# thangvubk/SoftGroup

Measured on AMD Instinct MI355X. Metric: scans/sec ScanNet-v2-like inference (softgroup_scannet.yaml, full forward_test), higher is better.
Workload: dtype f32

## Files before the change

### softgroup_amd/csrc/ballquery.hip

```cpp
#include "common.h"
#include "scan.h"

namespace sg {

constexpr int32_t kBqEmpty = 0x7f7f7f7f;
constexpr int kBqBuf = 2048;
constexpr int kBqCap = SG_BALLQUERY_MAX_NEIGHBORS;
constexpr int kBqKeep = 64;

struct BqWs {
  int4 *cell;
  int32_t *table;
  int32_t *count;
  int32_t *start;
  int32_t *cursor;
  int32_t *slot_of;
  float4 *sorted;
  int32_t *keep;
  void *scan_ws;
  size_t scan_bytes;
  uint32_t cap;
};

__device__ __forceinline__ uint32_t cell_slot(int b, int cx, int cy, int cz, uint32_t mask) {
  uint64_t h = (static_cast<uint64_t>(static_cast<uint32_t>(b)) << 32) | static_cast<uint32_t>(cx);
  h = mix64(h) ^ ((static_cast<uint64_t>(static_cast<uint32_t>(cy)) << 32) | static_cast<uint32_t>(cz));
  return static_cast<uint32_t>(mix64(h)) & mask;
}

__global__ void __launch_bounds__(256) bq_insert_kernel(const float *__restrict__ xyz,
                                                       const int32_t *__restrict__ batch_idxs,
                                                       int n, double inv_cell, int4 *__restrict__ cell,
                                                       int32_t *table, uint32_t mask, int32_t *count,
                                                       int32_t *__restrict__ slot_of) {
  const int i = blockIdx.x * 256 + threadIdx.x;
  if (i >= n) return;
  int4 c;
  c.x = batch_idxs ? batch_idxs[i] : 0;
  c.y = static_cast<int>(floor(static_cast<double>(xyz[3 * i + 0]) * inv_cell));
  c.z = static_cast<int>(floor(static_cast<double>(xyz[3 * i + 1]) * inv_cell));
  c.w = static_cast<int>(floor(static_cast<double>(xyz[3 * i + 2]) * inv_cell));
  cell[i] = c;
  uint32_t s = cell_slot(c.x, c.y, c.z, c.w, mask);
  while (true) {
    int32_t cur = __hip_atomic_load(&table[s], __ATOMIC_RELAXED, __HIP_MEMORY_SCOPE_AGENT);
    if (cur == kBqEmpty) {
      cur = atomicCAS(&table[s], kBqEmpty, i);
      if (cur == kBqEmpty) break;
    }
    int4 o;
    o.x = batch_idxs ? batch_idxs[cur] : 0;
    o.y = static_cast<int>(floor(static_cast<double>(xyz[3 * cur + 0]) * inv_cell));
    o.z = static_cast<int>(floor(static_cast<double>(xyz[3 * cur + 1]) * inv_cell));
    o.w = static_cast<int>(floor(static_cast<double>(xyz[3 * cur + 2]) * inv_cell));
    if (o.x == c.x && o.y == c.y && o.z == c.z && o.w == c.w) break;
    s = (s + 1) & mask;
  }
  slot_of[i] = static_cast<int32_t>(s);
  atomicAdd(&count[s], 1);
}

__global__ void __launch_bounds__(256) bq_scatter_kernel(const float *__restrict__ xyz, int n,
                                                        const int32_t *__restrict__ slot_of,
                                                        const int32_t *__restrict__ start,
                                                        int32_t *cursor, float4 *__restrict__ sorted) {
  const int i = blockIdx.x * 256 + threadIdx.x;
  if (i >= n) return;
  const int s = slot_of[i];
  const int pos = start[s] + atomicAdd(&cursor[s], 1);
  sorted[pos] = make_float4(xyz[3 * i], xyz[3 * i + 1], xyz[3 * i + 2], __int_as_float(i));
}

__device__ __forceinline__ float dist2(float ox, float oy, float oz, float x, float y, float z) {
  const float dx = __fsub_rn(ox, x), dy = __fsub_rn(oy, y), dz = __fsub_rn(oz, z);
  return __fmaf_rn(dz, dz, __fmaf_rn(dx, dx, __fmul_rn(dy, dy)));
}

struct BqCells {
  int start, excl, incl, total;
};
__device__ __forceinline__ BqCells bq_cells(int my_start, int my_count) {
  BqCells c;
  c.start = my_start;
  c.incl = wave_incl_scan(my_count);
  c.excl = c.incl - my_count;
  c.total = __shfl(c.incl, 63, 64);
  return c;
}
__device__ __forceinline__ int bq_candidate(const BqCells &c, int t) {
  int lo = 0, hi = 26;
#pragma unroll
  for (int it = 0; it < 5; ++it) {
    const int mid = (lo + hi) >> 1;
    const bool right = __shfl(c.incl, mid, 64) <= t;
    lo = right ? mid + 1 : lo;
    hi = right ? hi : mid;
  }
  return __shfl(c.start, lo, 64) + (t - __shfl(c.excl, lo, 64));
}

__device__ __forceinline__ int bq_scan_count(const float4 *__restrict__ sorted, const BqCells &c,
                                             float ox, float oy, float oz, float r2, int limit) {
  int total = 0;
  for (int t0 = 0; t0 < c.total; t0 += 64) {
    const int t = t0 + lane_id();
    const int at = bq_candidate(c, min(t, c.total - 1));
    if (t < c.total) {
      const float4 p = sorted[at];
      total += (dist2(ox, oy, oz, p.x, p.y, p.z) < r2 && __float_as_int(p.w) < limit) ? 1 : 0;
    }
  }
  return wave_sum(total);
}

template <bool FILL>
__global__ void __launch_bounds__(256) bq_query_kernel(const float *__restrict__ xyz, int n,
                                                      float r2, const int4 *__restrict__ cell,
                                                      const int32_t *__restrict__ table,
                                                      const int32_t *__restrict__ count,
                                                      const int32_t *__restrict__ start,
                                                      uint32_t mask, const float4 *__restrict__ sorted,
                                                      int32_t *__restrict__ start_len,
                                                      int32_t *__restrict__ idx_out, int32_t *__restrict__ keep) {
  __shared__ __attribute__((aligned(16))) int32_t buf_all[FILL ? 4 * kBqBuf : 4 * kBqKeep];
  const int wave = threadIdx.x >> 6, lane = threadIdx.x & 63;
  int32_t *buf = buf_all + wave * (FILL ? kBqBuf : kBqKeep);
  for (int i = blockIdx.x * 4 + wave; i < n; i += gridDim.x * 4) {
    if (FILL) {
      const int out_len = start_len[2 * i + 1];
      if (out_len <= kBqKeep) {
        if (lane < out_len) idx_out[static_cast<int64_t>(start_len[2 * i]) + lane] = keep[static_cast<int64_t>(i) * kBqKeep + lane];
        continue;
      }
    }
    const float ox = xyz[3 * i], oy = xyz[3 * i + 1], oz = xyz[3 * i + 2];
    const int4 c = cell[i];
    int my_start = 0, my_count = 0;
    if (lane < 27) {
      const int cx = c.y + lane / 9 - 1, cy = c.z + (lane / 3) % 3 - 1, cz = c.w + lane % 3 - 1;
      uint32_t s = cell_slot(c.x, cx, cy, cz, mask);
      while (true) {
        const int32_t rep = table[s];
        if (rep == kBqEmpty) break;
        const int4 o = cell[rep];
        if (o.x == c.x && o.y == cx && o.z == cy && o.w == cz) {
          my_start = start[s];
          my_count = count[s];
          break;
        }
        s = (s + 1) & mask;
      }
    }
    const BqCells cells = bq_cells(my_start, my_count);
    if (!FILL) {
      int m = 0;
      for (int t0 = 0; t0 < cells.total; t0 += 64) {
        const int t = t0 + lane;
        const int at = bq_candidate(cells, min(t, cells.total - 1));
        bool ok = false;
        int id = 0;
        if (t < cells.total) {
          const float4 p = sorted[at];
          id = __float_as_int(p.w);
          ok = dist2(ox, oy, oz, p.x, p.y, p.z) < r2;
        }
        const uint64_t bal = __ballot(ok);
        const int pos = m + mask_prefix(bal);
        if (ok && pos < kBqKeep) buf[pos] = id;
        m += __popcll(bal);
      }
      if (lane == 0) start_len[2 * i + 1] = min(m, kBqCap);
      if (m <= kBqKeep) {
        __builtin_amdgcn_fence(__ATOMIC_RELEASE, "wavefront");
        __builtin_amdgcn_wave_barrier();
        const int e = lane < m ? buf[lane] : 0x7fffffff;
        int rank = 0;
        for (int j = 0; j < m; ++j) rank += (buf[j] < e);
        if (lane < m) keep[static_cast<int64_t>(i) * kBqKeep + rank] = e;
      }
      __builtin_amdgcn_wave_barrier();
      continue;
    }
    const int out_start = start_len[2 * i], out_len = start_len[2 * i + 1];
    int limit = 0x7fffffff;
    int m = 0;
    for (int attempt = 0; attempt < 2; ++attempt) {
      m = 0;
      for (int t0 = 0; t0 < cells.total; t0 += 64) {
        const int t = t0 + lane;
        const int at = bq_candidate(cells, min(t, cells.total - 1));
        bool ok = false;
        int id = 0;
        if (t < cells.total) {
          const float4 p = sorted[at];
          id = __float_as_int(p.w);
          ok = dist2(ox, oy, oz, p.x, p.y, p.z) < r2 && id < limit;
        }
        const uint64_t bal = __ballot(ok);
        const int pos = m + mask_prefix(bal);
        if (ok && pos < kBqBuf) buf[pos] = id;
        m += __popcll(bal);
      }
      if (m <= kBqBuf) break;
      int lo = 0, hi = n;
      while (lo < hi) {
        const int mid = lo + (hi - lo) / 2;
        const int cmid = bq_scan_count(sorted, cells, ox, oy, oz, r2, mid);
        if (cmid >= out_len) hi = mid; else lo = mid + 1;
      }
      limit = lo;
    }
    __builtin_amdgcn_fence(__ATOMIC_RELEASE, "wavefront");
    __builtin_amdgcn_wave_barrier();
    for (int e0 = 0; e0 < m; e0 += 64) {
      const int ei = e0 + lane;
      const int e = ei < m ? buf[ei] : 0x7fffffff;
      int rank = 0;
      int j = 0;
      for (; j + 4 <= m; j += 4) {
        const int4 q = *reinterpret_cast<const int4 *>(buf + j);
        rank += (q.x < e) + (q.y < e) + (q.z < e) + (q.w < e);
      }
      for (; j < m; ++j) rank += (buf[j] < e);
      if (ei < m && rank < out_len) idx_out[static_cast<int64_t>(out_start) + rank] = e;
    }
    __builtin_amdgcn_wave_barrier();
  }
}

static size_t bq_cap(int n) {
  size_t cap = 1024;
  while (cap < static_cast<size_t>(n) * 2) cap <<= 1;
  return cap;
}

static bool bq_carve(void *ws, size_t ws_bytes, int n, BqWs *w) {
  Workspace a(ws, ws_bytes);
  const size_t nn = static_cast<size_t>(n > 0 ? n : 1);
  w->cap = static_cast<uint32_t>(bq_cap(n));
  w->cell = a.take<int4>(nn);
  w->sorted = a.take<float4>(nn);
  w->table = a.take<int32_t>(w->cap);
  w->count = a.take<int32_t>(w->cap);
  w->start = a.take<int32_t>(w->cap);
  w->cursor = a.take<int32_t>(w->cap);
  w->slot_of = a.take<int32_t>(nn);
  w->scan_bytes = scan_workspace_bytes(w->cap);
  w->scan_ws = a.take<char>(w->scan_bytes);
  w->keep = a.take<int32_t>(nn * kBqKeep);
  return w->scan_ws != nullptr && w->keep != nullptr;
}

}

using namespace sg;

extern "C" {

size_t sg_ballquery_workspace_bytes(int n) {
  const size_t nn = static_cast<size_t>(n > 0 ? n : 1);
  const size_t cap = bq_cap(n);
  return 2 * align_up(nn * 16) + 4 * align_up(cap * 4) + align_up(nn * 4) +
         align_up(scan_workspace_bytes(cap)) + align_up(nn * kBqKeep * 4) + 256;
}

int sg_ballquery_build_grid(const float *xyz, const int32_t *batch_idxs, int n, float radius,
                            void *ws, size_t ws_bytes, sg_stream_t stream_) {
  SG_REQUIRE(n >= 0 && radius > 0.f, "sg_ballquery_build_grid: bad arguments (n=%d r=%g)", n, radius);
  hipStream_t stream = as_stream(stream_);
  BqWs w;
  if (!bq_carve(ws, ws_bytes, n, &w)) {
    set_error("sg_ballquery_build_grid: workspace too small");
    return SG_ERR_WORKSPACE;
  }
  if (n == 0) return SG_OK;
  {
    FillList f;
    f.add(w.table, static_cast<size_t>(w.cap) * 4, 0x7f);
    f.add(w.count, static_cast<size_t>(w.cap) * 4, 0);
    f.add(w.cursor, static_cast<size_t>(w.cap) * 4, 0);
    fill_many(f, stream);
  }
  const double inv_cell = 1.0 / (static_cast<double>(radius) * (1.0 + 1e-6));
  const int grid = (n + 255) / 256;
  bq_insert_kernel<<<grid, 256, 0, stream>>>(xyz, batch_idxs, n, inv_cell, w.cell, w.table,
                                             w.cap - 1, w.count, w.slot_of);
  const int32_t *count = w.count;
  int32_t *start = w.start;
  auto in = [count] __device__(int64_t s) { return count[s]; };
  auto out = [start] __device__(int64_t s, int v) { start[s] = v; };
  int rc = exclusive_scan(in, out, w.cap, nullptr, w.scan_ws, w.scan_bytes, stream);
  if (rc != SG_OK) return rc;
  bq_scatter_kernel<<<grid, 256, 0, stream>>>(xyz, n, w.slot_of, w.start, w.cursor, w.sorted);
  return check_launch("sg_ballquery_build_grid");
}

int sg_ballquery_count(const float *xyz, const int32_t *batch_idxs, int n, float radius,
                       int32_t *start_len, int32_t *meta, void *ws, size_t ws_bytes,
                       sg_stream_t stream_) {
  (void)batch_idxs;
  (void)meta;
  SG_REQUIRE(n >= 0 && radius > 0.f, "sg_ballquery_count: bad arguments");
  BqWs w;
  if (!bq_carve(ws, ws_bytes, n, &w)) {
    set_error("sg_ballquery_count: workspace too small");
    return SG_ERR_WORKSPACE;
  }
  if (n == 0) return SG_OK;
  const float r2 = radius * radius;
  bq_query_kernel<false><<<grid_for(n, 4, 256 * 16), 256, 0, as_stream(stream_)>>>(
      xyz, n, r2, w.cell, w.table, w.count, w.start, w.cap - 1, w.sorted, start_len, nullptr, w.keep);
  return check_launch("sg_ballquery_count");
}

int sg_ballquery_fill(const float *xyz, const int32_t *batch_idxs, int n, float radius,
                      const int32_t *start_len, int32_t *idx, void *ws, size_t ws_bytes,
                      sg_stream_t stream_) {
  (void)batch_idxs;
  SG_REQUIRE(n >= 0 && radius > 0.f, "sg_ballquery_fill: bad arguments");
  BqWs w;
  if (!bq_carve(ws, ws_bytes, n, &w)) {
    set_error("sg_ballquery_fill: workspace too small");
    return SG_ERR_WORKSPACE;
  }
  if (n == 0) return SG_OK;
  const float r2 = radius * radius;
  bq_query_kernel<true><<<grid_for(n, 4, 256 * 16), 256, 0, as_stream(stream_)>>>(
      xyz, n, r2, w.cell, w.table, w.count, w.start, w.cap - 1, w.sorted,
      const_cast<int32_t *>(start_len), idx, w.keep);
  return check_launch("sg_ballquery_fill");
}

}
```

### softgroup_amd/csrc/bfs.hip

```cpp
#include <stdlib.h>

#include <map>
#include <mutex>
#include <utility>

#include "common.h"
#include "scan.h"

namespace sg {

constexpr int kCap = SG_BALLQUERY_MAX_NEIGHBORS;
constexpr int kEmitThreads = 512;
constexpr int kEmitWaves = kEmitThreads / 64;

#define SG_LD(p) __hip_atomic_load((p), __ATOMIC_RELAXED, __HIP_MEMORY_SCOPE_AGENT)
#define SG_ST(p, v) __hip_atomic_store((p), (v), __ATOMIC_RELAXED, __HIP_MEMORY_SCOPE_AGENT)

struct BfsWs {
  int32_t *parent, *lab, *size, *cid, *coff, *owner, *seeds, *ebase, *wcnt, *asym_nodes;
  int4 *label;
  int2 *erec;
  int32_t *counters;
  void *scan_ws;
  size_t scan_bytes;
// ... 1 lines not shown
  unsigned long long *big_rec[2];
};

constexpr int kBigFastWgs = 16;
constexpr int kBigSlice = 8192;
constexpr int kBigClusterMin = 16384;
inline bool big_fast_on() {
  const char *e = getenv("SG_BFS_BIG_FAST");
  return !(e && atoi(e) == 0);
}
inline int thin_levels_on() {
  const char *e = getenv("SG_BFS_THIN");
  return e ? atoi(e) : 0;
}
inline bool big_local_on() {
  const char *e = getenv("SG_BFS_BIG_LOCAL");
  return !(e && atoi(e) == 0);
}
inline size_t big_stage_entries(int n) {
  return n > kBigClusterMin && big_fast_on() ? static_cast<size_t>(n) + static_cast<size_t>(kBigFastWgs) * kBigSlice : 0;
}

static bool bfs_carve(void *ws, size_t ws_bytes, int n, int64_t n_edges, BfsWs *w) {
  Workspace a(ws, ws_bytes);
  const size_t nn = static_cast<size_t>(n > 0 ? n : 1);
  w->parent = a.take<int32_t>(nn);
  w->lab = a.take<int32_t>(nn);
  w->label = a.take<int4>(nn);
  w->size = a.take<int32_t>(nn);
  w->cid = a.take<int32_t>(nn);
  w->coff = a.take<int32_t>(nn);
  w->owner = a.take<int32_t>(nn);
  w->seeds = a.take<int32_t>(nn);
  w->ebase = a.take<int32_t>(nn);
  w->wcnt = a.take<int32_t>(nn);
  w->asym_nodes = a.take<int32_t>(nn);
  w->counters = a.take<int32_t>(64);
  w->scan_bytes = scan_workspace_bytes(n);
  w->scan_ws = a.take<char>(w->scan_bytes);
  w->erec = a.take<int2>(static_cast<size_t>(n_edges > 0 ? n_edges : 1));
  bool ok = w->scan_ws != nullptr && w->erec != nullptr;
  const size_t be = big_stage_entries(n);
  for (int i = 0; i < 2; ++i) {
    w->big_stage[i] = be ? a.take<int32_t>(be) : nullptr;
    w->big_rec[i] = be ? a.take<unsigned long long>(be) : nullptr;
    ok = ok && (be == 0 || (w->big_stage[i] != nullptr && w->big_rec[i] != nullptr));
  }
  return ok;
}

__device__ __forceinline__ int uf_find(int32_t *parent, int x) {
  int cur = SG_LD(&parent[x]);
  if (cur != x) {
    int prev = x, next;
    while (cur > (next = SG_LD(&parent[cur]))) {
      SG_ST(&parent[prev], next);
      prev = cur;
      cur = next;
    }
  }
  return cur;
}

__device__ __forceinline__ void uf_union(int32_t *parent, int a, int b) {
  while (a != b) {
    if (a < b) { const int t = a; a = b; b = t; }
    const int old = atomicCAS(&parent[a], a, b);
    if (old == a) return;
    a = uf_find(parent, old);
    b = uf_find(parent, b);
  }
}

__device__ __forceinline__ bool list_has_sorted(const int32_t *__restrict__ lst, int len, int key) {
  int lo = 0, hi = len;
  while (lo < hi) {
    const int mid = (lo + hi) >> 1;
    const int v = lst[mid];
    if (v < key) lo = mid + 1; else hi = mid;
  }
  return lo < len && lst[lo] == key;
}

__global__ void __launch_bounds__(256) bfs_init_kernel(int n, int32_t *parent, int32_t *size,
                                                      int32_t *owner) {
  const int i = blockIdx.x * 256 + threadIdx.x;
  if (i < n) {
    parent[i] = i;
    size[i] = 0;
    owner[i] = 0x7fffffff;
  }
}

constexpr int kSample = 2;
template <int SAMPLE>
__global__ void __launch_bounds__(256) bfs_union_kernel(const int32_t *__restrict__ idx,
                                                       const int32_t *__restrict__ start_len, int n,
                                                       int lists_sorted, int radius_lists,
                                                       int32_t *parent, int32_t *asym_nodes,
                                                       int32_t *counters) {
  const int wave = threadIdx.x >> 6, lane = threadIdx.x & 63;
  for (int u = blockIdx.x * 4 + wave; u < n; u += gridDim.x * 4) {
    const int st = start_len[2 * u], ln_all = start_len[2 * u + 1];
    const int ln = SAMPLE ? min(ln_all, kSample) : ln_all;
    const bool u_capped = ln_all >= kCap;
    bool any_asym = false;
    const int ru = SAMPLE ? -1 : SG_LD(&parent[u]);
    for (int p0 = 0; p0 < ln; p0 += 64) {
      const int p = p0 + lane;
      const int v = p < ln ? idx[st + p] : u;
      bool sym = true;
      if (v != u) {
        const int vst = start_len[2 * v], vln = start_len[2 * v + 1];
        if (!radius_lists || u_capped || vln >= kCap) {
          if (lists_sorted) {
            sym = list_has_sorted(idx + vst, vln, u);
          } else {
            sym = false;
            for (int j = 0; j < vln; ++j)
              if (idx[vst + j] == u) { sym = true; break; }
          }
        }
        if (sym) {
          if (v < u && (SAMPLE || SG_LD(&parent[v]) != ru)) uf_union(parent, uf_find(parent, u), uf_find(parent, v));
        }
      }
      any_asym |= !sym;
    }
    if (!SAMPLE && __any(any_asym)) {
      if (lane == 0) asym_nodes[atomicAdd(&counters[0], 1)] = u;
    }
  }
}

__global__ void __launch_bounds__(256) bfs_hook_min_kernel(const int32_t *__restrict__ idx,
                                                          const int32_t *__restrict__ start_len, int n,
                                                          int lists_sorted, int radius_lists, int32_t *parent) {
  const int u = blockIdx.x * 256 + threadIdx.x;
  if (u >= n) return;
  const int st = start_len[2 * u], ln = start_len[2 * u + 1];
  if (ln == 0 || !lists_sorted) return;
  const int v = idx[st];
  if (v >= u) return;
  if (!radius_lists || ln >= kCap || start_len[2 * v + 1] >= kCap)
    if (!list_has_sorted(idx + start_len[2 * v], start_len[2 * v + 1], u)) return;
  parent[u] = v;
}
__global__ void __launch_bounds__(256) bfs_compress_kernel(int n, int32_t *parent) {
  const int i = blockIdx.x * 256 + threadIdx.x;
  if (i < n) SG_ST(&parent[i], uf_find(parent, i));
}

__global__ void __launch_bounds__(256) bfs_flatten_kernel(int n, int32_t *parent, int32_t *lab) {
  const int i = blockIdx.x * 256 + threadIdx.x;
  if (i >= n) return;
  int r = i;
  while (true) {
    const int p = SG_LD(&parent[r]);
    if (p == r) break;
    r = p;
  }
  lab[i] = r;
}
__global__ void __launch_bounds__(256) bfs_store_root_kernel(int n, const int32_t *__restrict__ lab,
                                                            int32_t *__restrict__ parent) {
  const int i = blockIdx.x * 256 + threadIdx.x;
  if (i < n) parent[i] = lab[i];
}

__global__ void __launch_bounds__(256) bfs_propagate_kernel(const int32_t *__restrict__ idx,
                                                           const int32_t *__restrict__ start_len,
                                                           const int32_t *__restrict__ asym_nodes,
                                                           int n_asym,
                                                           const int32_t *__restrict__ root_of,
                                                           int32_t *lab, int32_t *counters) {
  const int wave = threadIdx.x >> 6, lane = threadIdx.x & 63;
  for (int a = blockIdx.x * 4 + wave; a < n_asym; a += gridDim.x * 4) {
    const int u = asym_nodes[a];
    const int ru = root_of[u];
    const int st = start_len[2 * u], ln = start_len[2 * u + 1];
    for (int p = lane; p < ln; p += 64) {
      const int rv = root_of[idx[st + p]];
      if (rv == ru) continue;
      const int lu = SG_LD(&lab[ru]);
      if (lu < SG_LD(&lab[rv])) {
        if (atomicMin(&lab[rv], lu) > lu) SG_ST(&counters[1], 1);
      }
    }
  }
}

__global__ void __launch_bounds__(256) bfs_label_kernel(int n, const int32_t *__restrict__ root_of,
                                                       const int32_t *__restrict__ lab,
                                                       const int32_t *__restrict__ start_len,
                                                       int4 *__restrict__ node_rec, int32_t *size) {
  const int i = blockIdx.x * 256 + threadIdx.x;
  const bool valid = i < n;
  const int l = valid ? lab[root_of[i]] : -1;
  int slot = 0;
  uint64_t todo = __ballot(valid);
  const int lane = threadIdx.x & 63;
  while (todo) {
    const int leader = __ffsll(static_cast<long long>(todo)) - 1;
    const int ll = __shfl(l, leader, 64);
    const uint64_t same = __ballot(valid && l == ll) & todo;
    int base = 0;
    if (lane == leader) base = atomicAdd(&size[ll], __popcll(same));
    base = __shfl(base, leader, 64);
    if ((same >> lane) & 1ull) slot = base + __popcll(same & ((1ull << lane) - 1ull));
    todo &= ~same;
  }
  if (!valid) return;
  node_rec[i] = make_int4(l, slot, start_len[2 * i], start_len[2 * i + 1]);
}

__global__ void __launch_bounds__(256) bfs_zero_size_kernel(int n, int32_t *size) {
  const int i = blockIdx.x * 256 + threadIdx.x;
  if (i < n) size[i] = 0;
}

__global__ void __launch_bounds__(256) bfs_owner_reset_kernel(int n, const int4 *__restrict__ label,
                                                             const int32_t *__restrict__ size,
                                                             int min_size, const int32_t *gate,
                                                             int32_t *__restrict__ owner) {
  if (SG_LD(gate) == 0) return;
  for (int i = blockIdx.x * 256 + threadIdx.x; i < n; i += gridDim.x * 256)
    if (size[label[i].x] > min_size) owner[i] = 0x7fffffff;
// ... 1321 lines not shown
    hipStreamDestroy(it->second.side);
    hipEventDestroy(it->second.fork);
    hipEventDestroy(it->second.join);
    hipEventDestroy(it->second.back);
  }
  g_bfs_side.erase(it);
}
struct BfsLabelNote {
  const void *ws = nullptr;
  int max_kept = -1;
};
static thread_local BfsLabelNote t_bfs_note;

void bfs_emit_defer(BfsDefer *d) { t_bfs_defer = d; }
int bfs_emit_join(const BfsDefer &d, hipStream_t stream) {
  if (!d.deferred) return SG_OK;
  BfsSide *side = bfs_side(stream);
  if (side == nullptr || side->side != d.side || hipEventRecord(side->join, side->side) != hipSuccess ||
      hipStreamWaitEvent(stream, side->join, 0) != hipSuccess) {
    set_error("bfs_emit_join: joining the side stream failed");
    return SG_ERR_LAUNCH;
  }
  return SG_OK;
}
int bfs_label_max_kept(const void *ws) { return t_bfs_note.ws == ws ? t_bfs_note.max_kept : -1; }

__global__ void __launch_bounds__(256) bfs_kept_members_kernel(const int32_t *__restrict__ l2p, int n_pts,
                                                              const int4 *__restrict__ label,
                                                              const int32_t *__restrict__ size,
                                                              const float *__restrict__ thr_dev,
                                                              int32_t *__restrict__ out) {
  __shared__ int wsum[4];
  const float thr = thr_dev[0];
  int mine = 0;
  for (int p = blockIdx.x * 256 + threadIdx.x; p < n_pts; p += gridDim.x * 256)
    mine += static_cast<float>(size[label[l2p[p]].x]) >= thr ? 1 : 0;
  const int w = wave_sum(mine);
  if ((threadIdx.x & 63) == 0) wsum[threadIdx.x >> 6] = w;
  __syncthreads();
  if (threadIdx.x == 0) atomicAdd(out, wsum[0] + wsum[1] + wsum[2] + wsum[3]);
}
int bfs_count_kept_members(const void *ws, size_t ws_bytes, int n, int64_t n_edges, const int32_t *l2p, int n_pts,
                           const float *thr_dev, int32_t *out, hipStream_t stream) {
  BfsWs w;
  if (!bfs_carve(const_cast<void *>(ws), ws_bytes, n, n_edges, &w)) {
    set_error("bfs_count_kept_members: workspace too small");
    return SG_ERR_WORKSPACE;
  }
  hipMemsetAsync(out, 0, 4, stream);
  bfs_kept_members_kernel<<<grid_for(n_pts, 256, 1024), 256, 0, stream>>>(l2p, n_pts, w.label, w.size, thr_dev, out);
  return check_launch("bfs_count_kept_members");
}

}

using namespace sg;

extern "C" {

size_t sg_bfs_workspace_bytes(int n, int64_t n_edges) {
  const size_t nn = static_cast<size_t>(n > 0 ? n : 1);
  const size_t ne = static_cast<size_t>(n_edges > 0 ? n_edges : 1);
  const size_t be = big_stage_entries(n);
  return 14 * align_up(nn * 4) + align_up(64 * 4) + align_up(scan_workspace_bytes(n)) +
         align_up(ne * sizeof(int2)) + 2 * (align_up(be * 4) + align_up(be * 8)) + 256;
}

int sg_bfs_cluster_label(const int32_t *bq_idxs, const int32_t *start_len, int n, int64_t n_edges,
                         int list_flags, const int32_t *seg_of_point, const float *seg_thr,
                         int n_seg, int32_t *n_cluster_host, int32_t *sum_npoint_host, void *ws,
                         size_t ws_bytes, sg_stream_t stream_) {
  SG_REQUIRE(n >= 0 && n_seg >= 1 && seg_thr != nullptr, "sg_bfs_cluster_label: bad arguments");
  hipStream_t stream = as_stream(stream_);
  BfsWs w;
  if (!bfs_carve(ws, ws_bytes, n, n_edges, &w)) {
    set_error("sg_bfs_cluster_label: workspace too small");
    return SG_ERR_WORKSPACE;
  }
  *n_cluster_host = 0;
  *sum_npoint_host = 0;
  if (n == 0) return SG_OK;
  const int grid = (n + 255) / 256;
  hipMemsetAsync(w.counters, 0, 64 * 4, stream);
  bfs_init_kernel<<<grid, 256, 0, stream>>>(n, w.parent, w.size, w.owner);
  static const bool one_pass = getenv("SG_BFS_ONE_PASS") != nullptr;
  if (!one_pass) {
    static const bool sample_env = getenv("SG_BFS_SAMPLE") != nullptr;
    if (sample_env || !(list_flags & SG_LISTS_SORTED))
      bfs_union_kernel<1><<<grid_for(n, 4, 256 * 16), 256, 0, stream>>>(bq_idxs, start_len, n,
                                                                      list_flags & SG_LISTS_SORTED,
                                                                      list_flags & SG_LISTS_RADIUS,
                                                                      w.parent, w.asym_nodes, w.counters);
    else
      bfs_hook_min_kernel<<<grid, 256, 0, stream>>>(bq_idxs, start_len, n, list_flags & SG_LISTS_SORTED,
                                                   list_flags & SG_LISTS_RADIUS, w.parent);
    bfs_compress_kernel<<<grid, 256, 0, stream>>>(n, w.parent);
  }
  bfs_union_kernel<0><<<grid_for(n, 4, 256 * 16), 256, 0, stream>>>(bq_idxs, start_len, n,
                                                                  list_flags & SG_LISTS_SORTED,
                                                                  list_flags & SG_LISTS_RADIUS,
                                                                  w.parent, w.asym_nodes, w.counters);
  bfs_flatten_kernel<<<grid, 256, 0, stream>>>(n, w.parent, w.lab);
  bfs_store_root_kernel<<<grid, 256, 0, stream>>>(n, w.lab, w.parent);

  int32_t *host_counters = pinned_words();
  SG_REQUIRE(host_counters != nullptr, "sg_bfs_cluster_label: pinned allocation failed");
  for (int i = 0; i < 5; ++i) host_counters[i] = 0;
  for (int pass = 0; pass < 2; ++pass) {
    if (pass == 1) {
      const int n_asym = host_counters[0];
      while (true) {
        hipMemsetAsync(w.counters + 1, 0, 4, stream);
        bfs_propagate_kernel<<<grid_for(n_asym, 4, 256 * 16), 256, 0, stream>>>(
            bq_idxs, start_len, w.asym_nodes, n_asym, w.parent, w.lab, w.counters);
        host_counters[8] = 0;
        hipMemcpyAsync(host_counters + 8, w.counters + 1, 4, hipMemcpyDeviceToHost, stream);
        if (hipStreamSynchronize(stream) != hipSuccess) return check_launch("bfs propagate");
        if (!host_counters[8]) break;
      }
      bfs_zero_size_kernel<<<grid, 256, 0, stream>>>(n, w.size);
    }
    bfs_label_kernel<<<grid, 256, 0, stream>>>(n, w.parent, w.lab, start_len, w.label, w.size);
    const int4 *label = w.label;
    const int32_t *size = w.size;
    int32_t *cid = w.cid, *coff = w.coff;
    auto keep = [label, size, seg_of_point, seg_thr] __device__(int64_t i) -> int {
      if (label[i].x != static_cast<int32_t>(i)) return 0;
      const float thr = seg_thr[seg_of_point ? seg_of_point[i] : 0];
      return static_cast<float>(size[i]) >= thr ? 1 : 0;
    };
    int32_t *max_kept = w.counters + 4;
    auto keep_size = [keep, size, max_kept] __device__(int64_t i) -> int {
      const int s = keep(i) ? size[i] : 0;
      if (s > kBigMin) atomicMax(max_kept, s);
      return s;
    };
    int rc = exclusive_scan(keep, [cid] __device__(int64_t i, int v) { cid[i] = v; }, n,
                            w.counters + 2, w.scan_ws, w.scan_bytes, stream);
    if (rc != SG_OK) return rc;
    rc = exclusive_scan(keep_size, [coff] __device__(int64_t i, int v) { coff[i] = v; }, n,
                        w.counters + 3, w.scan_ws, w.scan_bytes, stream);
    if (rc != SG_OK) return rc;
    hipMemcpyAsync(host_counters, w.counters, 5 * sizeof(int32_t), hipMemcpyDeviceToHost, stream);
    if (hipStreamSynchronize(stream) != hipSuccess) return check_launch("sg_bfs_cluster_label");
    if (host_counters[0] == 0) break;
    if (pass == 0) hipMemsetAsync(w.counters + 4, 0, 4, stream);
  }
  *n_cluster_host = host_counters[2];
  *sum_npoint_host = host_counters[3];
  t_bfs_note.ws = ws;
  t_bfs_note.max_kept = host_counters[4];
  return check_launch("sg_bfs_cluster_label");
}

int sg_bfs_cluster_emit(const int32_t *bq_idxs, const int32_t *start_len, int n, int64_t n_edges,
                        const int32_t *seg_of_point, const float *seg_thr, int n_cluster,
                        int sum_npoint, int32_t *cluster_idxs, int32_t *cluster_offsets, void *ws,
                        size_t ws_bytes, sg_stream_t stream_) {
  SG_REQUIRE(n >= 0 && n_cluster >= 0 && sum_npoint >= 0, "sg_bfs_cluster_emit: bad arguments");
  hipStream_t stream = as_stream(stream_);
  BfsWs w;
  if (!bfs_carve(ws, ws_bytes, n, n_edges, &w)) {
    set_error("sg_bfs_cluster_emit: workspace too small");
    return SG_ERR_WORKSPACE;
  }
  if (n_cluster == 0 || n == 0) {
    hipMemsetAsync(cluster_offsets, 0, 4, stream);
    return SG_OK;
  }
  bfs_seed_kernel<<<(n + 255) / 256, 256, 0, stream>>>(n, w.label, w.size, w.cid, w.coff,
                                                       seg_of_point, seg_thr, w.seeds,
                                                       cluster_offsets);
  bfs_edge_rec_kernel<<<grid_for(n, 4, 256 * 16), 256, 0, stream>>>(bq_idxs, w.label, w.cid, w.seeds, n,
                                                                     n_cluster, w.erec);
  static const bool want_stats = getenv("SG_BFS_STATS") != nullptr;
  int32_t *stats = nullptr;
  if (want_stats) {
    hipMalloc(&stats, 256 * 8 * 4);
// ... 135 lines not shown
```

### softgroup_amd/csrc/scan_forward.hip

```cpp
#include <stdlib.h>
#include <string.h>
#include <condition_variable>

#include <map>
#include <mutex>
#include <utility>

#include "common.h"
#include "heads.h"

#define SG_TRY_(expr)             \
  do {                            \
    const int rc_ = (expr);       \
    if (rc_ != SG_OK) return rc_; \
  } while (0)

namespace sg {

extern thread_local void (*t_scan_emit_hook)(void *);
extern thread_local void (*t_unet_conv_hook)(void *);
extern thread_local void *t_unet_conv_ctx;
extern thread_local void *t_scan_emit_ctx;

__global__ void __launch_bounds__(256) voxelize_cat_kernel(const float *__restrict__ a, int ca,
// ... 232 lines not shown
static void start_dense_copy(void *ctx) {
  DenseCopy *d = static_cast<DenseCopy *>(ctx);
  if (d->issued || d->bytes == 0) return;
  d->issued = true;
  static const int d2h_wgs = getenv("SG_SCAN_D2H_WGS") ? atoi(getenv("SG_SCAN_D2H_WGS")) : 0;
  static const bool side = !(getenv("SG_SCAN_COPY_STREAM") && atoi(getenv("SG_SCAN_COPY_STREAM")) == 0);
  hipStream_t cs = side ? d->ss->copy : d->main;
  if (side && (hipEventRecord(d->ss->packed, d->main) != hipSuccess ||
               hipStreamWaitEvent(d->ss->copy, d->ss->packed, 0) != hipSuccess)) {
    d->failed = true;
    return;
  }
  if (d2h_wgs > 0 && d->bytes % 16 == 0) {
    d2h_copy_kernel<<<d2h_wgs, 256, 0, cs>>>(static_cast<const u32x4 *>(d->dev_block),
                                             static_cast<u32x4 *>(d->host_block), d->bytes / 16);
    if (hipGetLastError() != hipSuccess) d->failed = true;
  } else if (hipMemcpyAsync(d->host_block, d->dev_block, d->bytes, hipMemcpyDeviceToHost, cs) != hipSuccess) {
    d->failed = true;
  }
  if (hipEventRecord(d->ss->copied, cs) != hipSuccess) d->failed = true;
}

static Mlp2 as_mlp(const sg_mlp2 &m) { return Mlp2{m.w1, m.b1, m.bn_scale, m.bn_shift, m.w2, m.b2, m.out}; }

struct Carve {
  char *base;
  size_t cap, off;
  Carve(void *p, size_t n) : base(static_cast<char *>(p)), cap(n), off(0) {}
  template <typename T>
  T *take(size_t count) {
    const size_t bytes = align_up((count ? count : 1) * sizeof(T));
    const size_t at = off;
    off += bytes;
    return off > cap ? nullptr : reinterpret_cast<T *>(base + at);
  }
  size_t at(const void *p) const { return static_cast<size_t>(static_cast<const char *>(p) - base); }
};

}

using namespace sg;

extern "C" {

int sg_softmax_rows(const float *x, int64_t rows, int cols, float *out, sg_stream_t stream) {
  SG_REQUIRE(rows >= 0 && cols >= 1 && cols <= 32 && x && out, "sg_softmax_rows: rows of 1..32 columns (got %d)", cols);
  if (rows == 0) return SG_OK;
  const int grid = static_cast<int>((rows + 255) / 256);
  if (cols <= 4) softmax_rows_kernel<4><<<grid, 256, 0, as_stream(stream)>>>(x, rows, cols, out);
  else if (cols <= 8) softmax_rows_kernel<8><<<grid, 256, 0, as_stream(stream)>>>(x, rows, cols, out);
  else if (cols <= 16) softmax_rows_kernel<16><<<grid, 256, 0, as_stream(stream)>>>(x, rows, cols, out);
  else softmax_rows_kernel<32><<<grid, 256, 0, as_stream(stream)>>>(x, rows, cols, out);
  return check_launch("sg_softmax_rows");
}

int sg_mlp_rows(const float *feats, const int32_t *idx, int64_t rows, int channels, const sg_mlp2 *mlp, float *out,
                sg_stream_t stream) {
  SG_REQUIRE(rows >= 0 && mlp && feats && out, "sg_mlp_rows: bad arguments");
  SG_REQUIRE(channels == 16 || channels == 32, "sg_mlp_rows: channels must be 16 or 32 (got %d)", channels);
  SG_REQUIRE(mlp->out >= 1 && mlp->out <= 32, "sg_mlp_rows: head width %d out of range", mlp->out);
  if (rows == 0) return SG_OK;
  const int grid = static_cast<int>((rows + 255) / 256);
  if (channels == 32) mlp_rows_kernel<32><<<grid, 256, 0, as_stream(stream)>>>(feats, idx, rows, as_mlp(*mlp), out);
  else mlp_rows_kernel<16><<<grid, 256, 0, as_stream(stream)>>>(feats, idx, rows, as_mlp(*mlp), out);
  return check_launch("sg_mlp_rows");
}

int sg_linear_rows(const float *x, int64_t rows, const sg_linear *lin, float *out, sg_stream_t stream) {
  SG_REQUIRE(rows >= 0 && lin && lin->w && lin->out >= 1 && lin->in >= 1 && x && out, "sg_linear_rows: bad arguments");
  if (rows == 0) return SG_OK;
  linear_rows_kernel<<<grid_for(rows * lin->out, 256), 256, 0, as_stream(stream)>>>(x, rows, lin->w, lin->b, lin->out,
                                                                                  lin->in, out);
  return check_launch("sg_linear_rows");
}

size_t sg_scan_arena_bytes(const sg_scan_desc *d, int n_points, int n_voxels) {
  if (d == nullptr || d->backbone == nullptr) return 0;
  const size_t N = static_cast<size_t>(n_points > 0 ? n_points : 1), M = static_cast<size_t>(n_voxels > 0 ? n_voxels : 1);
  const size_t C = static_cast<size_t>(d->channels), ns = static_cast<size_t>(d->semantic_classes);
  size_t p = align_up(M * 16) + align_up(M * 8 * 4) + align_up(M * C * 4) + align_up(N * C * 4) + 2 * align_up(N * ns * 4) +
             align_up(N * 12) + 2 * align_up(N * 8) + align_up(N * 96) + (1 << 20);
  size_t bb = sg_unet_arena_bytes(d->backbone, n_voxels) / 4;
  if (bb < (64u << 20)) bb = 64u << 20;
  const size_t later = (160u << 20) + N * 256;
  return p + (bb > later ? bb : later) + (8 << 20);
}

int sg_scan_forward(const sg_scan_desc *d, const sg_scan_input *in, void *arena, size_t arena_bytes, void *host_dense,
                    size_t host_dense_bytes, void *host_inst, size_t host_inst_bytes, sg_scan_result *res,
                    sg_stream_t stream_) {
  static const char *kWhat = "sg_scan_forward";
  SG_REQUIRE(d && in && res && d->backbone, "sg_scan_forward: null descriptor");
  SG_REQUIRE(!d->want_instances || d->tiny, "sg_scan_forward: instances need the tiny U-Net's descriptor");
  SG_REQUIRE(d->channels == 16 || d->channels == 32, "sg_scan_forward: backbone channels must be 16 or 32");
  SG_REQUIRE(d->semantic.out == d->semantic_classes && d->semantic_classes >= 1 && d->semantic_classes <= 32,
             "sg_scan_forward: 1..32 semantic classes");
  SG_REQUIRE(in->n_points >= 0 && in->n_voxels >= 0 && in->max_active >= 0 && in->batch_size >= 1 && in->feat_dim >= 1,
             "sg_scan_forward: bad input sizes");
  SG_REQUIRE(in->n_dense >= 0 && in->n_dense <= SG_SCAN_DENSE_MAX, "sg_scan_forward: at most %d dense items",
             SG_SCAN_DENSE_MAX);
  memset(res, 0, sizeof(*res));
  hipStream_t stream = as_stream(stream_);
  const int N = in->n_points, M = in->n_voxels, C = d->channels, ns = d->semantic_classes;
  const int cin = in->feat_dim + (d->with_coords ? 3 : 0);
  SG_REQUIRE(d->backbone->input_w == nullptr ? cin == C : cin == d->backbone->input_cin,
             "sg_scan_forward: %d feature columns, the backbone takes %d", cin,
             d->backbone->input_w ? d->backbone->input_cin : C);
  if (N == 0 || M == 0) return SG_OK;
  ScanStream *ss = scan_stream(stream);
  SG_REQUIRE(ss != nullptr, "sg_scan_forward: side stream / event creation failed");
  Carve ar(arena, arena_bytes);
#define SG_CARVE(var, T, count)                                                                          \
  T *var = ar.take<T>(count);                                                                            \
  if (var == nullptr) {                                                                                  \
    res->arena_needed = ar.off + ar.off / 4 + (64u << 20);                                               \
    set_error("%s: arena too small (%zu bytes, need about %zu)", kWhat, ar.cap, res->arena_needed);      \
    return SG_ERR_WORKSPACE;                                                                             \
  }

  const int32_t *vc32 = static_cast<const int32_t *>(in->voxel_coords);
  if (in->voxel_coords_is_int64) {
    SG_CARVE(vc, int32_t, static_cast<size_t>(M) * 4);
    narrow_i64_kernel<<<grid_for(static_cast<int64_t>(M) * 4, 256), 256, 0, stream>>>(
        static_cast<const int64_t *>(in->voxel_coords), static_cast<int64_t>(M) * 4, vc);
    vc32 = vc;
  }
  SG_CARVE(vfeat, float, static_cast<size_t>(M) * cin);
  SG_CARVE(bb_out, float, static_cast<size_t>(M) * C);
  SG_CARVE(out_feats, float, static_cast<size_t>(N) * C);
  SG_CARVE(sem, float, static_cast<size_t>(N) * ns);
  SG_CARVE(prob, float, static_cast<size_t>(N) * ns);
  SG_CARVE(off, float, static_cast<size_t>(N) * 3);
  SG_CARVE(preds, int64_t, N);
  PackList pl;
  pl.n = 0;
  size_t dense_total = 0;
  bool want_gt = false;
  for (int i = 0; i < in->n_dense; ++i) {
    const sg_scan_dense_item &it = in->dense[i];
    size_t nb = 0;
    switch (it.kind) {
      case 0: nb = it.bytes; SG_REQUIRE(it.ptr != nullptr || nb == 0, "sg_scan_forward: dense item %d has no source", i); break;
      case 1: nb = static_cast<size_t>(N) * 8; break;
      case 2: nb = static_cast<size_t>(N) * 12; break;
      case 3:
        nb = static_cast<size_t>(N) * 8;
        want_gt = true;
        SG_REQUIRE(in->semantic_labels && in->instance_labels, "sg_scan_forward: gt_instances need the label arrays");
        break;
      case 4: nb = static_cast<size_t>(N) * ns * 4; break;
      default: SG_REQUIRE(false, "sg_scan_forward: dense item %d: unknown kind %d", i, it.kind);
    }
    res->dense_offset[i] = dense_total;
    pl.dst[i] = dense_total;
    pl.bytes[i] = nb;
    dense_total += align_up(nb);
  }
  pl.n = in->n_dense;
  res->dense_bytes = dense_total;
  res->host_dense_needed = dense_total;
  if (dense_total > 0 && (host_dense == nullptr || host_dense_bytes < dense_total)) {
    set_error("%s: host block for the dense results too small (%zu bytes, need %zu)", kWhat, host_dense_bytes, dense_total);
    return SG_ERR_WORKSPACE;
  }
  int64_t *gt = nullptr;
  if (want_gt) {
    SG_CARVE(gt_, int64_t, N);
// ... 212 lines not shown
```

Before: 421.0.

## Precompute per-cell neighbor rows and batch short-list fill and union passes

Adds a build-time kernel that, for each occupied grid cell, precomputes the 27 neighbor cell starts and prefix counts, so each query no longer repeats the hash probing. The count pass now walks points in cell-sorted order for locality, and the fill pass handles 16 points per wave when every list is short. The BFS union gains a batched path that skips symmetry checks when no list hit the cap, tracked through a new global flag. The cost is extra arena memory, one more kernel launch, and more code complexity.

After: 417.9. No clear change (-0.7%).

```diff
diff --git a/softgroup_amd/csrc/ballquery.hip b/softgroup_amd/csrc/ballquery.hip
--- a/softgroup_amd/csrc/ballquery.hip
+++ b/softgroup_amd/csrc/ballquery.hip
@@ -7,6 +7,8 @@
 constexpr int kBqBuf = 2048;
 constexpr int kBqCap = SG_BALLQUERY_MAX_NEIGHBORS;
 constexpr int kBqKeep = 64;
+constexpr int kBqRow = 28;
+constexpr int kBqFillBatch = 16;
 
 struct BqWs {
   int4 *cell;
@@ -17,6 +19,8 @@
   int32_t *slot_of;
   float4 *sorted;
   int32_t *keep;
+  int2 *rows;
+  int32_t *row_of;
   void *scan_ws;
   size_t scan_bytes;
   uint32_t cap;
@@ -63,12 +67,51 @@
 __global__ void __launch_bounds__(256) bq_scatter_kernel(const float *__restrict__ xyz, int n,
                                                         const int32_t *__restrict__ slot_of,
                                                         const int32_t *__restrict__ start,
-                                                        int32_t *cursor, float4 *__restrict__ sorted) {
+                                                        int32_t *cursor, float4 *__restrict__ sorted,
+                                                        int32_t *__restrict__ row_of) {
   const int i = blockIdx.x * 256 + threadIdx.x;
   if (i >= n) return;
   const int s = slot_of[i];
-  const int pos = start[s] + atomicAdd(&cursor[s], 1);
+  const int first = start[s];
+  const int pos = first + atomicAdd(&cursor[s], 1);
   sorted[pos] = make_float4(xyz[3 * i], xyz[3 * i + 1], xyz[3 * i + 2], __int_as_float(i));
+  row_of[pos] = first;
+}
+
+__global__ void __launch_bounds__(256) bq_cell_rows_kernel(int n, const int4 *__restrict__ cell,
+                                                          const int32_t *__restrict__ table,
+                                                          const int32_t *__restrict__ count,
+                                                          const int32_t *__restrict__ start, uint32_t mask,
+                                                          const float4 *__restrict__ sorted,
+                                                          const int32_t *__restrict__ row_of,
+                                                          int2 *__restrict__ rows) {
+  const int64_t tid = static_cast<int64_t>(blockIdx.x) * 256 + threadIdx.x;
+  const int j = static_cast<int>(tid >> 5), k = threadIdx.x & 31;
+  const bool rep = j < n && row_of[j] == j;
+  int my_start = 0, my_count = 0;
+  if (rep && k < 27) {
+    const int4 c = cell[__float_as_int(sorted[j].w)];
+    const int cx = c.y + k / 9 - 1, cy = c.z + (k / 3) % 3 - 1, cz = c.w + k % 3 - 1;
+    uint32_t s = cell_slot(c.x, cx, cy, cz, mask);
+    while (true) {
+      const int32_t r = table[s];
+      if (r == kBqEmpty) break;
+      const int4 o = cell[r];
+      if (o.x == c.x && o.y == cx && o.z == cy && o.w == cz) {
+        my_start = start[s];
+        my_count = count[s];
+        break;
+      }
+      s = (s + 1) & mask;
+    }
+  }
+  int incl = my_count;
+#pragma unroll
+  for (int o = 1; o < 32; o <<= 1) {
+    const int up = __shfl_up(incl, o, 32);
+    if (k >= o) incl += up;
+  }
+  if (rep && k < kBqRow) rows[static_cast<int64_t>(j) * kBqRow + k] = make_int2(my_start, incl);
 }
 
 __device__ __forceinline__ float dist2(float ox, float oy, float oz, float x, float y, float z) {
@@ -79,12 +122,15 @@
 struct BqCells {
   int start, excl, incl, total;
 };
-__device__ __forceinline__ BqCells bq_cells(int my_start, int my_count) {
+__device__ __forceinline__ BqCells bq_cells(const int2 *__restrict__ rows, int row) {
+  const int lane = lane_id();
+  const int2 e = lane < kBqRow ? rows[static_cast<int64_t>(row) * kBqRow + lane] : make_int2(0, 0);
   BqCells c;
-  c.start = my_start;
-  c.incl = wave_incl_scan(my_count);
-  c.excl = c.incl - my_count;
-  c.total = __shfl(c.incl, 63, 64);
+  c.start = e.x;
+  c.incl = e.y;
+  const int prev = __shfl_up(e.y, 1, 64);
+  c.excl = lane == 0 ? 0 : prev;
+  c.total = __shfl(e.y, 26, 64);
   return c;
 }
 __device__ __forceinline__ int bq_candidate(const BqCells &c, int t) {
@@ -113,46 +159,37 @@
   return wave_sum(total);
 }
 
+__device__ __forceinline__ int bq_batch_node(int incl, int t) {
+  int lo = 0, hi = kBqFillBatch - 1;
+#pragma unroll
+  for (int it = 0; it < 4; ++it) {
+    const int mid = (lo + hi) >> 1;
+    const bool right = __shfl(incl, mid, 64) <= t;
+    lo = right ? mid + 1 : lo;
+    hi = right ? hi : mid;
+  }
+  return lo;
+}
+static_assert(kBqFillBatch == 16, "bq_batch_node searches 16 prefixes in 4 steps");
+
 template <bool FILL>
 __global__ void __launch_bounds__(256) bq_query_kernel(const float *__restrict__ xyz, int n,
-                                                      float r2, const int4 *__restrict__ cell,
-                                                      const int32_t *__restrict__ table,
-                                                      const int32_t *__restrict__ count,
+                                                      float r2, const int32_t *__restrict__ slot_of,
                                                       const int32_t *__restrict__ start,
-                                                      uint32_t mask, const float4 *__restrict__ sorted,
+                                                      const int2 *__restrict__ rows,
+                                                      const int32_t *__restrict__ row_of,
+                                                      const float4 *__restrict__ sorted,
                                                       int32_t *__restrict__ start_len,
                                                       int32_t *__restrict__ idx_out, int32_t *__restrict__ keep) {
   __shared__ __attribute__((aligned(16))) int32_t buf_all[FILL ? 4 * kBqBuf : 4 * kBqKeep];
   const int wave = threadIdx.x >> 6, lane = threadIdx.x & 63;
   int32_t *buf = buf_all + wave * (FILL ? kBqBuf : kBqKeep);
-  for (int i = blockIdx.x * 4 + wave; i < n; i += gridDim.x * 4) {
-    if (FILL) {
-      const int out_len = start_len[2 * i + 1];
-      if (out_len <= kBqKeep) {
-        if (lane < out_len) idx_out[static_cast<int64_t>(start_len[2 * i]) + lane] = keep[static_cast<int64_t>(i) * kBqKeep + lane];
-        continue;
-      }
-    }
-    const float ox = xyz[3 * i], oy = xyz[3 * i + 1], oz = xyz[3 * i + 2];
-    const int4 c = cell[i];
-    int my_start = 0, my_count = 0;
-    if (lane < 27) {
-      const int cx = c.y + lane / 9 - 1, cy = c.z + (lane / 3) % 3 - 1, cz = c.w + lane % 3 - 1;
-      uint32_t s = cell_slot(c.x, cx, cy, cz, mask);
-      while (true) {
-        const int32_t rep = table[s];
-        if (rep == kBqEmpty) break;
-        const int4 o = cell[rep];
-        if (o.x == c.x && o.y == cx && o.z == cy && o.w == cz) {
-          my_start = start[s];
-          my_count = count[s];
-          break;
-        }
-        s = (s + 1) & mask;
-      }
-    }
-    const BqCells cells = bq_cells(my_start, my_count);
-    if (!FILL) {
+  if (!FILL) {
+    for (int j = blockIdx.x * 4 + wave; j < n; j += gridDim.x * 4) {
+      const float4 q = sorted[j];
+      const int i = __float_as_int(q.w);
+      const float ox = q.x, oy = q.y, oz = q.z;
+      const BqCells cells = bq_cells(rows, row_of[j]);
       int m = 0;
       for (int t0 = 0; t0 < cells.total; t0 += 64) {
         const int t = t0 + lane;
@@ -175,56 +212,89 @@
         __builtin_amdgcn_wave_barrier();
         const int e = lane < m ? buf[lane] : 0x7fffffff;
         int rank = 0;
-        for (int j = 0; j < m; ++j) rank += (buf[j] < e);
+        for (int jj = 0; jj < m; ++jj) rank += (buf[jj] < e);
         if (lane < m) keep[static_cast<int64_t>(i) * kBqKeep + rank] = e;
       }
       __builtin_amdgcn_wave_barrier();
+    }
+    return;
+  }
+  const int n_batches = (n + kBqFillBatch - 1) / kBqFillBatch;
+  for (int b = blockIdx.x * 4 + wave; b < n_batches; b += gridDim.x * 4) {
+    const int u0 = b * kBqFillBatch, nb = min(kBqFillBatch, n - u0);
+    int b_st = 0, b_ln = 0;
+    if (lane < nb) {
+      const int2 sl = *reinterpret_cast<const int2 *>(start_len + 2 * static_cast<int64_t>(u0 + lane));
+      b_st = sl.x;
+      b_ln = sl.y;
+    }
+    if (!__any(b_ln > kBqKeep)) {
+      const int incl = wave_incl_scan(b_ln);
+      const int excl = incl - b_ln;
+      const int total = __builtin_amdgcn_readlane(incl, 63);
+      for (int t0 = 0; t0 < total; t0 += 64) {
+        const int t = t0 + lane;
+        const int tc = min(t, total - 1);
+        const int k = bq_batch_node(incl, tc);
+        const int p = tc - __shfl(excl, k, 64);
+        const int64_t dst = static_cast<int64_t>(__shfl(b_st, k, 64)) + p;
+        if (t < total) idx_out[dst] = keep[static_cast<int64_t>(u0 + k) * kBqKeep + p];
+      }
       continue;
     }
-    const int out_start = start_len[2 * i], out_len = start_len[2 * i + 1];
-    int limit = 0x7fffffff;
-    int m = 0;
-    for (int attempt = 0; attempt < 2; ++attempt) {
-      m = 0;
-      for (int t0 = 0; t0 < cells.total; t0 += 64) {
-        const int t = t0 + lane;
-        const int at = bq_candidate(cells, min(t, cells.total - 1));
-        bool ok = false;
-        int id = 0;
-        if (t < cells.total) {
-          const float4 p = sorted[at];
-          id = __float_as_int(p.w);
-          ok = dist2(ox, oy, oz, p.x, p.y, p.z) < r2 && id < limit;
+    for (int k = 0; k < nb; ++k) {
+      const int i = u0 + k;
+      const int out_start = __shfl(b_st, k, 64), out_len = __shfl(b_ln, k, 64);
+      if (out_len <= kBqKeep) {
+        if (lane < out_len) idx_out[static_cast<int64_t>(out_start) + lane] = keep[static_cast<int64_t>(i) * kBqKeep + lane];
+        continue;
+      }
+      const float ox = xyz[3 * i], oy = xyz[3 * i + 1], oz = xyz[3 * i + 2];
+      const BqCells cells = bq_cells(rows, start[slot_of[i]]);
+      int limit = 0x7fffffff;
+      int m = 0;
+      for (int attempt = 0; attempt < 2; ++attempt) {
+        m = 0;
+        for (int t0 = 0; t0 < cells.total; t0 += 64) {
+          const int t = t0 + lane;
+          const int at = bq_candidate(cells, min(t, cells.total - 1));
+          bool ok = false;
+          int id = 0;
+          if (t < cells.total) {
+            const float4 p = sorted[at];
+            id = __float_as_int(p.w);
+            ok = dist2(ox, oy, oz, p.x, p.y, p.z) < r2 && id < limit;
+          }
+          const uint64_t bal = __ballot(ok);
+          const int pos = m + mask_prefix(bal);
+          if (ok && pos < kBqBuf) buf[pos] = id;
+          m += __popcll(bal);
         }
-        const uint64_t bal = __ballot(ok);
-        const int pos = m + mask_prefix(bal);
-        if (ok && pos < kBqBuf) buf[pos] = id;
-        m += __popcll(bal);
-      }
-      if (m <= kBqBuf) break;
-      int lo = 0, hi = n;
-      while (lo < hi) {
-        const int mid = lo + (hi - lo) / 2;
-        const int cmid = bq_scan_count(sorted, cells, ox, oy, oz, r2, mid);
-        if (cmid >= out_len) hi = mid; else lo = mid + 1;
-      }
-      limit = lo;
-    }
-    __builtin_amdgcn_fence(__ATOMIC_RELEASE, "wavefront");
-    __builtin_amdgcn_wave_barrier();
-    for (int e0 = 0; e0 < m; e0 += 64) {
-      const int ei = e0 + lane;
-      const int e = ei < m ? buf[ei] : 0x7fffffff;
-      int rank = 0;
-      int j = 0;
-      for (; j + 4 <= m; j += 4) {
-        const int4 q = *reinterpret_cast<const int4 *>(buf + j);
-        rank += (q.x < e) + (q.y < e) + (q.z < e) + (q.w < e);
-      }
-      for (; j < m; ++j) rank += (buf[j] < e);
-      if (ei < m && rank < out_len) idx_out[static_cast<int64_t>(out_start) + rank] = e;
-    }
-    __builtin_amdgcn_wave_barrier();
+        if (m <= kBqBuf) break;
+        int lo = 0, hi = n;
+        while (lo < hi) {
+          const int mid = lo + (hi - lo) / 2;
+          const int cmid = bq_scan_count(sorted, cells, ox, oy, oz, r2, mid);
+          if (cmid >= out_len) hi = mid; else lo = mid + 1;
+        }
+        limit = lo;
+      }
+      __builtin_amdgcn_fence(__ATOMIC_RELEASE, "wavefront");
+      __builtin_amdgcn_wave_barrier();
+      for (int e0 = 0; e0 < m; e0 += 64) {
+        const int ei = e0 + lane;
+        const int e = ei < m ? buf[ei] : 0x7fffffff;
+        int rank = 0;
+        int j = 0;
+        for (; j + 4 <= m; j += 4) {
+          const int4 q = *reinterpret_cast<const int4 *>(buf + j);
+          rank += (q.x < e) + (q.y < e) + (q.z < e) + (q.w < e);
+        }
+        for (; j < m; ++j) rank += (buf[j] < e);
+        if (ei < m && rank < out_len) idx_out[static_cast<int64_t>(out_start) + rank] = e;
+      }
+      __builtin_amdgcn_wave_barrier();
+    }
   }
 }
 
@@ -248,7 +318,9 @@
   w->scan_bytes = scan_workspace_bytes(w->cap);
   w->scan_ws = a.take<char>(w->scan_bytes);
   w->keep = a.take<int32_t>(nn * kBqKeep);
-  return w->scan_ws != nullptr && w->keep != nullptr;
+  w->rows = a.take<int2>(nn * kBqRow);
+  w->row_of = a.take<int32_t>(nn);
+  return w->scan_ws != nullptr && w->keep != nullptr && w->rows != nullptr && w->row_of != nullptr;
 }
 
 }
@@ -261,7 +333,8 @@
   const size_t nn = static_cast<size_t>(n > 0 ? n : 1);
   const size_t cap = bq_cap(n);
   return 2 * align_up(nn * 16) + 4 * align_up(cap * 4) + align_up(nn * 4) +
-         align_up(scan_workspace_bytes(cap)) + align_up(nn * kBqKeep * 4) + 256;
+         align_up(scan_workspace_bytes(cap)) + align_up(nn * kBqKeep * 4) + align_up(nn * kBqRow * 8) +
+         align_up(nn * 4) + 256;
 }
 
 int sg_ballquery_build_grid(const float *xyz, const int32_t *batch_idxs, int n, float radius,
@@ -291,7 +364,10 @@
   auto out = [start] __device__(int64_t s, int v) { start[s] = v; };
   int rc = exclusive_scan(in, out, w.cap, nullptr, w.scan_ws, w.scan_bytes, stream);
   if (rc != SG_OK) return rc;
-  bq_scatter_kernel<<<grid, 256, 0, stream>>>(xyz, n, w.slot_of, w.start, w.cursor, w.sorted);
+  bq_scatter_kernel<<<grid, 256, 0, stream>>>(xyz, n, w.slot_of, w.start, w.cursor, w.sorted, w.row_of);
+  const int row_grid = static_cast<int>((static_cast<int64_t>(n) * 32 + 255) / 256);
+  bq_cell_rows_kernel<<<row_grid, 256, 0, stream>>>(n, w.cell, w.table, w.count, w.start, w.cap - 1, w.sorted,
+                                                   w.row_of, w.rows);
   return check_launch("sg_ballquery_build_grid");
 }
 
@@ -309,7 +385,7 @@
   if (n == 0) return SG_OK;
   const float r2 = radius * radius;
   bq_query_kernel<false><<<grid_for(n, 4, 256 * 16), 256, 0, as_stream(stream_)>>>(
-      xyz, n, r2, w.cell, w.table, w.count, w.start, w.cap - 1, w.sorted, start_len, nullptr, w.keep);
+      xyz, n, r2, w.slot_of, w.start, w.rows, w.row_of, w.sorted, start_len, nullptr, w.keep);
   return check_launch("sg_ballquery_count");
 }
 
@@ -325,9 +401,8 @@
   }
   if (n == 0) return SG_OK;
   const float r2 = radius * radius;
-  bq_query_kernel<true><<<grid_for(n, 4, 256 * 16), 256, 0, as_stream(stream_)>>>(
-      xyz, n, r2, w.cell, w.table, w.count, w.start, w.cap - 1, w.sorted,
-      const_cast<int32_t *>(start_len), idx, w.keep);
+  bq_query_kernel<true><<<grid_for((n + kBqFillBatch - 1) / kBqFillBatch, 4, 256 * 16), 256, 0, as_stream(stream_)>>>(
+      xyz, n, r2, w.slot_of, w.start, w.rows, w.row_of, w.sorted, const_cast<int32_t *>(start_len), idx, w.keep);
   return check_launch("sg_ballquery_fill");
 }
 
diff --git a/softgroup_amd/csrc/bfs.hip b/softgroup_amd/csrc/bfs.hip
--- a/softgroup_amd/csrc/bfs.hip
+++ b/softgroup_amd/csrc/bfs.hip
@@ -107,15 +107,32 @@
   return lo < len && lst[lo] == key;
 }
 
-__global__ void __launch_bounds__(256) bfs_init_kernel(int n, int32_t *parent, int32_t *size,
-                                                      int32_t *owner) {
+constexpr int kCappedWord = 5;
+__global__ void __launch_bounds__(256) bfs_init_kernel(int n, const int32_t *__restrict__ start_len,
+                                                      int32_t *parent, int32_t *size, int32_t *owner,
+                                                      int32_t *counters) {
   const int i = blockIdx.x * 256 + threadIdx.x;
   if (i < n) {
     parent[i] = i;
     size[i] = 0;
     owner[i] = 0x7fffffff;
-  }
-}
+    if (start_len[2 * i + 1] >= kCap) counters[kCappedWord] = 1;
+  }
+}
+
+constexpr int kUnionBatch = 16;
+__device__ __forceinline__ int union_batch_node(int incl, int t) {
+  int lo = 0, hi = kUnionBatch - 1;
+#pragma unroll
+  for (int it = 0; it < 4; ++it) {
+    const int mid = (lo + hi) >> 1;
+    const bool right = __shfl(incl, mid, 64) <= t;
+    lo = right ? mid + 1 : lo;
+    hi = right ? hi : mid;
+  }
+  return lo;
+}
+static_assert(kUnionBatch == 16, "union_batch_node searches 16 prefixes in 4 steps");
 
 constexpr int kSample = 2;
 template <int SAMPLE>
@@ -125,6 +142,34 @@
                                                        int32_t *parent, int32_t *asym_nodes,
                                                        int32_t *counters) {
   const int wave = threadIdx.x >> 6, lane = threadIdx.x & 63;
+  const bool any_capped = __builtin_amdgcn_readfirstlane(counters[kCappedWord]) != 0;
+  if (!SAMPLE && radius_lists && lists_sorted && !any_capped) {
+    const int n_batches = (n + kUnionBatch - 1) / kUnionBatch;
+    for (int b = blockIdx.x * 4 + wave; b < n_batches; b += gridDim.x * 4) {
+      const int u0 = b * kUnionBatch, nb = min(kUnionBatch, n - u0);
+      int b_st = 0, b_ln = 0, b_ru = 0;
+      if (lane < nb) {
+        const int2 sl = *reinterpret_cast<const int2 *>(start_len + 2 * static_cast<int64_t>(u0 + lane));
+        b_st = sl.x;
+        b_ln = sl.y;
+        b_ru = SG_LD(&parent[u0 + lane]);
+      }
+      const int incl = wave_incl_scan(b_ln);
+      const int excl = incl - b_ln;
+      const int total = __builtin_amdgcn_readlane(incl, 63);
+      for (int t0 = 0; t0 < total; t0 += 64) {
+        const int t = t0 + lane;
+        const int tc = min(t, total - 1);
+        const int k = union_batch_node(incl, tc);
+        const int64_t at = static_cast<int64_t>(__shfl(b_st, k, 64)) + (tc - __shfl(excl, k, 64));
+        const int ru = __shfl(b_ru, k, 64);
+        const int u = u0 + k;
+        const int v = t < total ? idx[at] : u;
+        if (v < u && SG_LD(&parent[v]) != ru) uf_union(parent, uf_find(parent, u), uf_find(parent, v));
+      }
+    }
+    return;
+  }
   for (int u = blockIdx.x * 4 + wave; u < n; u += gridDim.x * 4) {
     const int st = start_len[2 * u], ln_all = start_len[2 * u + 1];
     const int ln = SAMPLE ? min(ln_all, kSample) : ln_all;
@@ -136,8 +181,8 @@
       const int v = p < ln ? idx[st + p] : u;
       bool sym = true;
       if (v != u) {
-        const int vst = start_len[2 * v], vln = start_len[2 * v + 1];
-        if (!radius_lists || u_capped || vln >= kCap) {
+        if (!radius_lists || (any_capped && (u_capped || start_len[2 * v + 1] >= kCap))) {
+          const int vst = start_len[2 * v], vln = start_len[2 * v + 1];
           if (lists_sorted) {
             sym = list_has_sorted(idx + vst, vln, u);
           } else {
@@ -160,14 +205,16 @@
 
 __global__ void __launch_bounds__(256) bfs_hook_min_kernel(const int32_t *__restrict__ idx,
                                                           const int32_t *__restrict__ start_len, int n,
-                                                          int lists_sorted, int radius_lists, int32_t *parent) {
+                                                          int lists_sorted, int radius_lists, int32_t *parent,
+                                                          const int32_t *__restrict__ counters) {
   const int u = blockIdx.x * 256 + threadIdx.x;
   if (u >= n) return;
+  const bool any_capped = counters[kCappedWord] != 0;
   const int st = start_len[2 * u], ln = start_len[2 * u + 1];
   if (ln == 0 || !lists_sorted) return;
   const int v = idx[st];
   if (v >= u) return;
-  if (!radius_lists || ln >= kCap || start_len[2 * v + 1] >= kCap)
+  if (!radius_lists || (any_capped && (ln >= kCap || start_len[2 * v + 1] >= kCap)))
     if (!list_has_sorted(idx + start_len[2 * v], start_len[2 * v + 1], u)) return;
   parent[u] = v;
 }
@@ -1655,7 +1702,7 @@
   if (n == 0) return SG_OK;
   const int grid = (n + 255) / 256;
   hipMemsetAsync(w.counters, 0, 64 * 4, stream);
-  bfs_init_kernel<<<grid, 256, 0, stream>>>(n, w.parent, w.size, w.owner);
+  bfs_init_kernel<<<grid, 256, 0, stream>>>(n, start_len, w.parent, w.size, w.owner, w.counters);
   static const bool one_pass = getenv("SG_BFS_ONE_PASS") != nullptr;
   if (!one_pass) {
     static const bool sample_env = getenv("SG_BFS_SAMPLE") != nullptr;
@@ -1666,7 +1713,7 @@
                                                                       w.parent, w.asym_nodes, w.counters);
     else
       bfs_hook_min_kernel<<<grid, 256, 0, stream>>>(bq_idxs, start_len, n, list_flags & SG_LISTS_SORTED,
-                                                   list_flags & SG_LISTS_RADIUS, w.parent);
+                                                   list_flags & SG_LISTS_RADIUS, w.parent, w.counters);
     bfs_compress_kernel<<<grid, 256, 0, stream>>>(n, w.parent);
   }
   bfs_union_kernel<0><<<grid_for(n, 4, 256 * 16), 256, 0, stream>>>(bq_idxs, start_len, n,
diff --git a/softgroup_amd/csrc/scan_forward.hip b/softgroup_amd/csrc/scan_forward.hip
--- a/softgroup_amd/csrc/scan_forward.hip
+++ b/softgroup_amd/csrc/scan_forward.hip
@@ -338,7 +338,7 @@
              align_up(N * 12) + 2 * align_up(N * 8) + align_up(N * 96) + (1 << 20);
   size_t bb = sg_unet_arena_bytes(d->backbone, n_voxels) / 4;
   if (bb < (64u << 20)) bb = 64u << 20;
-  const size_t later = (160u << 20) + N * 256;
+  const size_t later = (160u << 20) + N * 512;
   return p + (bb > later ? bb : later) + (8 << 20);
 }
 
```
